# TheCacophonyProject/audio-analysis

Measured on AMD Instinct MI355X. Metric: audio-seconds classified/sec/GPU on 60 s mono; max|delta logit| vs CPU ref, higher is better.
Workload: dtype bf16x3; 1 GPU; config2: 64 windows/step (39 of clip A + 25 of clip B, 60 s 48 kHz mono), htk log-mel n_fft 4096 hop 640 160 mel + model1 CNN; model=model1, global_batch=64, seq_len=144000, parallelism=dp1, pipeline=2 batches in flight on 2 streams, clip_pairs=4 resident clip pairs in rotation, one per step

## Files before the change

audio-analysis_amd/csrc/aa_cnn.hip:

```cpp
#include "aa_common.h"

#include <cmath>
#include <cstdlib>
#include <cstring>
#include <string>
#include <type_traits>
#include <vector>

namespace aa {

typedef __attribute__((ext_vector_type(8))) __bf16 bf16x8;
typedef __attribute__((ext_vector_type(4))) float f32x4;
typedef __attribute__((ext_vector_type(2))) float f32x2;
typedef __attribute__((ext_vector_type(16))) float f32x16;
typedef __bf16 bf16;
struct fp8 {
    uint8_t v;
};
struct bf16x3 {};

template <typename T>
struct Prec {
    using L = T;
    using G = T;
// ... 819 lines not shown
            for (int o = 0; o < 8; ++o)
                if (o < nc) best[o] = fmaxf(best[o], apply_act(acc[o] + bias[c0 + o], act, alpha));
        }
    TO* dst = out + ((size_t)(n * Hout + oh) * Wout + ow) * cout + c0;
    for (int o = 0; o < nc; ++o) dst[o] = to_t<TO>(best[o]);
}

template <typename TI>
__global__ __launch_bounds__(256) void pool_dense(const TI* __restrict__ in, int HW, int C,
                                                  const float* __restrict__ w, const float* __restrict__ b, int U,
                                                  int sigmoid, float* __restrict__ logits, float* __restrict__ probs) {
    extern __shared__ float mx[];
    const int n = blockIdx.x;
    const TI* src = in + (size_t)n * HW * C;
    for (int c = threadIdx.x; c < C; c += blockDim.x) {
        float m = -INFINITY;
        for (int p = 0; p < HW; ++p) m = fmaxf(m, to_f(src[(size_t)p * C + c]));
        mx[c] = m;
    }
    __syncthreads();
    for (int u = threadIdx.x; u < U; u += blockDim.x) {
        float v;
        if (w) {
            v = 0.f;
            for (int c = 0; c < C; ++c) v = fmaf(mx[c], w[(size_t)c * U + u], v);
            v += b[u];
        } else {
            v = mx[u];
        }
        logits[(size_t)n * U + u] = v;
        if (probs) probs[(size_t)n * U + u] = sigmoid ? 1.f / (1.f + expf(-v)) : v;
    }
}

__global__ void track_mean(const float* __restrict__ probs, int n_models, long long model_stride, int L,
                           const int* __restrict__ wb, const int* __restrict__ wc,
                           float* __restrict__ out) {
    const int t = blockIdx.x;
    const int c = threadIdx.x;
    if (c >= L) return;
    constexpr int U = 40;
    float acc = 0.f;
    const int n = wc[t];
    const float* base = probs + (size_t)wb[t] * L + c;
    for (int w0 = 0; w0 < n; w0 += U) {
        float m[U];
#pragma unroll
        for (int u = 0; u < U; ++u) m[u] = 0.f;
        for (int k = 0; k < n_models; ++k) {
            float v[U];
#pragma unroll
            for (int u = 0; u < U; ++u) v[u] = base[k * model_stride + (size_t)min(w0 + u, n - 1) * L];
#pragma unroll
            for (int u = 0; u < U; ++u) m[u] = __fadd_rn(m[u], v[u]);
        }
#pragma unroll
        for (int u = 0; u < U; ++u)
            if (w0 + u < n) acc = __fadd_rn(acc, __fdiv_rn(m[u], (float)n_models));
    }
    out[(size_t)t * L + c] = n > 0 ? __fdiv_rn(acc, (float)n) : NAN;
}

}

#include "aa_conv_x3.h"
#include "aa_conv_wg.h"
#include "aa_gconv.h"
#include "aa_conv_tail.h"

namespace aa {

template <int MODE>
__global__ void stage_decode(const void* __restrict__ src, float* __restrict__ dst, size_t total, int cout) {
    for (size_t i = (size_t)blockIdx.x * blockDim.x + threadIdx.x; i < total; i += (size_t)gridDim.x * blockDim.x) {
        float v;
        if (MODE == 0) {
            v = static_cast<const float*>(src)[i];
        } else if (MODE == 1) {
            v = __uint_as_float((uint32_t) static_cast<const uint16_t*>(src)[i] << 16);
        } else if (MODE == 2) {
            const uint32_t b = static_cast<const uint8_t*>(src)[i];
            const int e = (b >> 3) & 15, m = b & 7;
            const float a = (e == 15 && m == 7) ? __uint_as_float(0x7fc00000u)
                            : e == 0            ? ldexpf((float)m, -9)
                                                : ldexpf((float)(8 + m), e - 10);
            v = (b & 0x80) ? -a : a;
        } else {
            const size_t pix = i / (size_t)cout;
            const int c = (int)(i - pix * (size_t)cout);
            const uint16_t* h = static_cast<const uint16_t*>(src) + pix * (size_t)cout * 2 + (size_t)(c >> 5) * 64 + (c & 31);
            v = __uint_as_float((uint32_t)h[0] << 16) + __uint_as_float((uint32_t)h[32] << 16);
        }
        dst[i] = v;
    }
}

}

#include "aa_cnn_plan.h"

namespace aa {

template <typename Launch>
static int launch_tuned(const Stage& s, const Stage* first, int n, const void* kernel, size_t lds, bool window32,
                        int pool, int th, int tw, int bn, Launch&& launch) {
    if (window32)
        AA_CHECK((double)s.Hin * s.Win * s.cin * 4 < 2147483647.0, AA_ERR_UNSUPPORTED,
                 "conv %s: one window's activations exceed 2 GiB", s.name.c_str());
    FirstConv fc{};
    if (first) {
        const float slope = first->act == ACT_LEAKY ? first->alpha : first->act == ACT_RELU ? 0.f : 1.f;
        fc = FirstConv{(const float*)first->d_w, first->d_b, first->act, slope, first->has_mag,
                       first->mag_exp, first->Hin, first->Win, s.lm_f16};
    }
    AA_CHECK(lds <= 160 * 1024, AA_ERR_UNSUPPORTED, "conv %s: %zu B LDS", s.name.c_str(), lds);
    AA_DYN_LDS(kernel, lds);
    const int tiles_h = (s.Hout * pool + th - 1) / th;
    const int tiles_w = (s.Wout * pool + tw - 1) / tw;
    launch(dim3(tiles_h * tiles_w, s.cout_pad / bn, n), tiles_w, fc);
    AA_LAUNCH_CHECK();
    return AA_OK;
}

template <typename T, int KH, int KW, int CIN, int WM, int WN, int MF, int NF, int POOL, int TH, int TW,
          bool FUSED = false, bool EBF16 = false, int OCC = 0>
static int launch_mfma(const Stage& s, const void* in, void* out, int n, hipStream_t st,
                       const Stage* first = nullptr) {
    auto k = conv_mfma<T, KH, KW, CIN, WM, WN, MF, NF, POOL, TH, TW, FUSED, 0, EBF16, OCC>;
    constexpr int BN = WN * NF * 16;
    const size_t lds = conv_lds_bytes<T, KH, KW, CIN, BN, TH, TW, FUSED, EBF16>();
    using GT = typename Prec<T>::G;
    using LT = typename Prec<T>::L;
    return launch_tuned(s, FUSED ? first : nullptr, n, (const void*)k, lds, false, POOL, TH, TW, BN,
                        [&](dim3 grid, int tiles_w, const FirstConv& fc) {
        hipLaunchKernelGGL(k, grid, dim3(WM * WN * 64), lds, st, (const GT*)in, s.Hin, s.Win, (const LT*)s.d_w, s.d_b,
                           (GT*)out, s.Hout, s.Wout, s.cout, tiles_w, s.act, s.alpha, fc);
    });
}

template <int KH, int KW, int CIN, int WM, int WN, int MF, int NF, int POOL, int TH, int TW, bool RING, bool AJIT,
          int OCC, bool FUSED, bool IN_SPLIT, bool OUT_SPLIT>
static int launch_x3(const Stage& s, const void* in, void* out, int n, hipStream_t st, const Stage* first) {
    auto k = conv_x3<KH, KW, CIN, WM, WN, MF, NF, POOL, TH, TW, FUSED, 0, RING, AJIT, OCC, IN_SPLIT, OUT_SPLIT>;
    constexpr int BN = WN * NF * 16;
    const size_t lds = x3_lds_bytes<KH, KW, CIN, BN, TH, TW, FUSED, RING>();
    return launch_tuned(s, FUSED ? first : nullptr, n, (const void*)k, lds, true, POOL, TH, TW, BN,
                        [&](dim3 grid, int tiles_w, const FirstConv& fc) {
        hipLaunchKernelGGL(k, grid, dim3(WM * WN * 64), lds, st, (const float*)in, s.Hin, s.Win, (const bf16*)s.d_w,
                           s.d_b, (float*)out, s.Hout, s.Wout, s.cout, tiles_w, s.act, s.alpha, fc);
    });
}

template <int KH, int CIN, int WM, int WN, int MF, int NF, int POOL, int TH, int TW, int OCC, int WO, int NPASS,
          int BD, bool IN_SPLIT, bool OUT_SPLIT>
static int launch_wg(const Stage& s, const void* in, void* out, int n, hipStream_t st) {
    auto k = conv_wg<KH, CIN, WM, WN, MF, NF, POOL, TH, TW, OCC, IN_SPLIT, OUT_SPLIT, 0, WO, NPASS, BD>;
    constexpr int BN = WN * NF * 16;
    const size_t lds = wg_lds_bytes<KH, BN, TH, TW, WO, NPASS, WN>();
    return launch_tuned(s, nullptr, n, (const void*)k, lds, true, POOL, TH, TW, BN,
                        [&](dim3 grid, int tiles_w, const FirstConv&) {
        hipLaunchKernelGGL(k, grid, dim3(WM * WN * 64), lds, st, (const float*)in, s.Hin, s.Win, (const bf16*)s.d_w,
                           s.d_b, (float*)out, s.Hout, s.Wout, s.cout, tiles_w, s.act, s.alpha);
    });
}

template <bool CAN_FUSE, typename F>
static int dispatch_split(const Stage& s, F&& f) {
    using Y = std::true_type;
    using N = std::false_type;
    if constexpr (CAN_FUSE) {
        if (s.fused_first) return s.out_split ? f(Y{}, N{}, Y{}) : f(Y{}, N{}, N{});
    }
    if (s.in_split) return s.out_split ? f(N{}, Y{}, Y{}) : f(N{}, Y{}, N{});
    return s.out_split ? f(N{}, N{}, Y{}) : f(N{}, N{}, N{});
}

template <typename T>
static int launch_stage(const Model& m, const Stage& s, const void* in, void* out, float* logits,
                        float* probs, int n, hipStream_t st, const Stage* first, float* tmp) {
    using GT = typename Prec<T>::G;
    if (s.kind == ST_SMALL) {
        dim3 grid((s.Hc * s.Wc + 255) / 256, n);
        hipLaunchKernelGGL((conv_small<GT, 3, 3, 32>), grid, dim3(256), 0, st, (const float*)in, s.Hin,
                           s.Win, (const float*)s.d_w, s.d_b, s.has_mag, s.mag_exp, (GT*)out, s.Hc, s.Wc,
                           s.act, s.alpha);
        AA_LAUNCH_CHECK();
        return AA_OK;
    }
    if (s.kind == ST_GCONV) {
        if constexpr (!is_split<T>()) {
            set_error("%s: the runtime-shaped MFMA conv is split-bf16 only", s.name.c_str());
            return AA_ERR_UNSUPPORTED;
        } else {
            const ConvGeom g{s.Hin, s.Win, s.cin, s.Hc, s.Wc, s.cout, s.kh, s.kw, 1, 1, 0, 0, s.cin_pad};
            const bool pooled = s.ph > 1 || s.pw > 1;
            float* conv_out = pooled ? tmp : static_cast<float*>(out);
            const int gact_ = s.act == ACT_LEAKY ? GACT_LEAKY : s.act == ACT_RELU ? GACT_RELU : GACT_NONE;
            hipLaunchKernelGGL((gconv_x3t<2, 2, 2, 2>), dim3((s.Hc * s.Wc + 63) / 64, s.cout_pad / 64, n), dim3(256), 0, st,
                               (const float*)in, (const uint16_t*)s.d_w, s.d_b, conv_out, g, s.cout_pad, gact_,
                               s.alpha, nullptr, nullptr);
            AA_LAUNCH_CHECK();
            if (pooled) {
                const size_t items = (size_t)s.Hout * s.Wout * s.cout;
                hipLaunchKernelGGL(gpool2d, dim3((unsigned)((items + 255) / 256), n), dim3(256), 0, st, tmp,
                                   (float*)out, s.Hc, s.Wc, s.cout, s.Hout, s.Wout, s.ph, s.pw, s.ph, s.pw, 0, 0, 0,
                                   GACT_NONE, 0.f);
                AA_LAUNCH_CHECK();
            }
            return AA_OK;
        }
    }
    if (s.kind == ST_GENERIC) {
        if constexpr (is_fp8<T>()) {
            set_error("%s: no fp8 kernel for this shape", s.name.c_str());
            return AA_ERR_UNSUPPORTED;
        } else {
            dim3 grid((s.Hout * s.Wout + 255) / 256, (s.cout + 7) / 8, n);
            if (s.is_first) {
                hipLaunchKernelGGL((conv_generic<float, GT>), grid, dim3(256), 0, st, (const float*)in, s.Hin,
                                   s.Win, s.cin, (const float*)s.d_w, s.d_b, s.kh, s.kw, s.cout, s.ph, s.pw, s.Hout,
                                   s.Wout, s.act, s.alpha, s.has_mag, s.mag_exp, (GT*)out);
            } else {
                hipLaunchKernelGGL((conv_generic<GT, GT>), grid, dim3(256), 0, st, (const GT*)in, s.Hin, s.Win,
                                   s.cin, (const float*)s.d_w, s.d_b, s.kh, s.kw, s.cout, s.ph, s.pw, s.Hout,
                                   s.Wout, s.act, s.alpha, 0, 1.f, (GT*)out);
            }
            AA_LAUNCH_CHECK();
            return AA_OK;
        }
    }
    if (s.kind == ST_POOLDENSE) {
        hipLaunchKernelGGL((pool_dense<GT>), dim3(n), dim3(256), (size_t)s.cin * sizeof(float), st, (const GT*)in,
                           s.Hin * s.Win, s.cin, (const float*)s.d_w, s.d_b, s.cout, s.sigmoid, logits, probs);
        AA_LAUNCH_CHECK();
        return AA_OK;
    }
    if (s.kind == ST_HEAD && s.tail) {
        if constexpr (is_split<T>()) {
            const Stage& c = *first;
            const int tiles_h = (c.Hc + TAIL_TH - 1) / TAIL_TH, tiles_w = (c.Wc + TAIL_TW - 1) / TAIL_TW;
            auto k = conv_tail_x3<1, 3, 128, AA_TAIL_MF, TAIL_TH, TAIL_TW>;
            constexpr size_t lds = tail_lds_bytes<1, 3, 128, TAIL_TH, TAIL_TW>();
            AA_DYN_LDS(k, lds);
            float* part = static_cast<float*>(out);
            hipLaunchKernelGGL(k, dim3(tiles_h * tiles_w, 1, n), dim3(TAIL_NW * 64), lds, st, (const float*)in, c.Hin,
                               c.Win, (const bf16*)c.d_w, c.d_b, c.Hc, c.Wc, tiles_w, c.act, c.alpha,
                               (const bf16*)s.d_tw, part);
            AA_LAUNCH_CHECK();
            hipLaunchKernelGGL(head_final, dim3(n), dim3(64), 0, st, part, tiles_h * tiles_w, 32, s.d_b, s.cout, s.act,
                               s.alpha, s.sigmoid, logits, probs, (const float*)nullptr);
            AA_LAUNCH_CHECK();
            return AA_OK;
        } else {
            set_error("%s: the fused tail is split-bf16 only", s.name.c_str());
            return AA_ERR_UNSUPPORTED;
        }
    }
    if (s.kind == ST_HEAD) {
        const int HW = s.Hin * s.Win, parts = (HW + 63) / 64;
        float* part = static_cast<float*>(out);
        const float* hsc = is_fp8<T>() ? s.d_b + s.cout_pad : nullptr;
        hipLaunchKernelGGL((conv_head<GT, 1, 2>), dim3(n, parts, s.cout_pad / 32), dim3(256), 0, st, (const GT*)in,
                           HW, s.cin, (const GT*)s.d_w, s.d_b, s.cout, s.act, s.alpha, s.sigmoid, logits, probs, part,
                           hsc);
        AA_LAUNCH_CHECK();
        hipLaunchKernelGGL(head_final, dim3(n), dim3(s.cout <= 64 ? 64 : 256), 0, st, part, parts, s.cout_pad, s.d_b,
                           s.cout, s.act, s.alpha, s.sigmoid, logits, probs, hsc);
        AA_LAUNCH_CHECK();
        return AA_OK;
    }
    if (s.fused_first) {
        AA_CHECK(s.kh == 3 && s.kw == 3 && s.cin == 32 && s.pool == 3, AA_ERR_UNSUPPORTED,
                 "no fused first-layer kernel for %s", s.name.c_str());
    }
    if constexpr (is_split<T>()) {
        if (s.wg) {
#define AA_LAUNCHW(KH, CIN, POOL, WM, WN, MF, NF, TH, TW, OCC, WO, NPASS, BD)                                    \
            if (s.kh == KH && s.cin == CIN && s.pool == POOL)                                                    \
                return dispatch_split<false>(s, [&](auto, auto is, auto os) {                                    \
                    return launch_wg<KH, CIN, WM, WN, MF, NF, POOL, TH, TW, OCC, WO, NPASS, BD, decltype(is)::value, \
                                     decltype(os)::value>(s, in, out, n, st);                                    \
                });
            AA_WG_CFGS(AA_LAUNCHW)
#undef AA_LAUNCHW
            set_error("conv %dx%d cin %d pool %d: no Winograd kernel instantiation", s.kh, s.kw, s.cin, s.pool);
            return AA_ERR_UNSUPPORTED;
        }
#define AA_LAUNCH3(KH, KW, CIN, POOL, WM, WN, MF, NF, TH, TW, RING, AJIT, OCC)                                   \
        if (s.kh == KH && s.kw == KW && s.cin == CIN && s.pool == POOL)                                          \
            return dispatch_split<CIN == 32 && KH == 3 && KW == 3>(s, [&](auto fu, auto is, auto os) {           \
                return launch_x3<KH, KW, CIN, WM, WN, MF, NF, POOL, TH, TW, RING, AJIT, OCC, decltype(fu)::value, \
                                 decltype(is)::value, decltype(os)::value>(s, in, out, n, st, first);            \
            });
        AA_X3_CFGS(AA_LAUNCH3)
#undef AA_LAUNCH3
        set_error("conv %dx%d cin %d pool %d: no split-bf16 kernel instantiation", s.kh, s.kw, s.cin, s.pool);
        return AA_ERR_UNSUPPORTED;
    }
#define AA_LAUNCH(T_, KH, KW, CIN, POOL, WM, WN, MF, NF, TH, TW, EB, OCC)                                        \
    if constexpr (std::is_same<T, T_>::value) {                                                          \
        if (s.kh == KH && s.kw == KW && s.cin == CIN && s.pool == POOL) {                                \
            if (s.fused_first) {                                                                         \
                if constexpr (CIN == 32 && KH == 3 && KW == 3)                                           \
                    return launch_mfma<T, KH, KW, CIN, WM, WN, MF, NF, POOL, TH, TW, true, EB, OCC>(s, in, out, \
                                                                                              n, st, first); \
            } else {                                                                                     \
                return launch_mfma<T, KH, KW, CIN, WM, WN, MF, NF, POOL, TH, TW, false, EB, OCC>(s, in, out, n, st); \
            }                                                                                            \
        }                                                                                                \
    }
    AA_CONV_CFGS(AA_LAUNCH)
#undef AA_LAUNCH
    set_error("conv %dx%d cin %d pool %d: no kernel instantiation", s.kh, s.kw, s.cin, s.pool);
    return AA_ERR_UNSUPPORTED;
}

static void free_model(Model* m) {
    if (!m) return;
    m->timer.release();
    if (m->uploaded)
        for (auto& s : m->st) {
            (void)hipFree(s.d_w);
            (void)hipFree(s.d_b);
            (void)hipFree(s.d_tw);
        }
    delete m;
}

static int upload_model(Model* m) {
    m->uploaded = true;
    auto put = [](void** d, const void* h, size_t bytes) {
        hipError_t e = hipMalloc(d, bytes ? bytes : 4);
        if (e == hipSuccess && bytes) e = hipMemcpy(*d, h, bytes, hipMemcpyHostToDevice);
        return e;
    };
    for (Stage& s : m->st) {
        hipError_t e = s.h_w.empty() ? hipSuccess : put(&s.d_w, s.h_w.data(), s.h_w.size());
        if (e == hipSuccess) e = put((void**)&s.d_b, s.h_b.data(), sizeof(float) * s.h_b.size());
        AA_CHECK(e == hipSuccess, AA_ERR_HIP, "aa_model_create: layer %d: %s", s.layer_end, hipGetErrorString(e));
        if (!s.h_tw.empty()) e = put(&s.d_tw, s.h_tw.data(), s.h_tw.size());
        AA_CHECK(e == hipSuccess, AA_ERR_HIP, "aa_model_create: %s", hipGetErrorString(e));
        std::vector<uint8_t>().swap(s.h_w);
        std::vector<uint8_t>().swap(s.h_tw);
        std::vector<float>().swap(s.h_b);
    }
    return AA_OK;
}

template <typename T>
static int run_stages_t(Model* m, const void* x, int n, int last_stage, float* logits, float* probs, void* workspace,
                        hipStream_t st, bool timed, const void** last_out) {
    const size_t es = prec_bytes(m->prec);
    char* buf[2] = {static_cast<char*>(workspace),
                    static_cast<char*>(workspace) + align_up(m->act_elems[0] * es * n, 256)};
    float* tmp = reinterpret_cast<float*>(buf[1] + align_up(m->act_elems[1] * es * n, 256));
    const void* in = x;
    for (int k = 0; k <= last_stage; ++k) {
        const Stage& s = m->st[k];
        if (s.skipped) continue;
        void* out = buf[(s.tail ? k - 1 : k) % 2];
        const Stage* first = (s.fused_first || s.tail) ? &m->st[k - 1] : nullptr;
        hipEvent_t e0 = nullptr;
        int rc = timed ? m->timer.begin(k, st, &e0) : AA_OK;
        if (rc != AA_OK) return rc;
        rc = launch_stage<T>(*m, s, in, out, logits, probs, n, st, first, tmp);
        if (rc != AA_OK) return rc;
        rc = m->timer.end(k, st, e0);
        if (rc != AA_OK) return rc;
        in = out;
    }
    if (last_out) *last_out = in;
    return AA_OK;
}

static int run_stages(Model* m, const void* x, int n, int last_stage, float* logits, float* probs, void* workspace,
                      hipStream_t st, bool timed, const void** last_out = nullptr) {
    switch (m->prec) {
        case AA_PREC_BF16: return run_stages_t<bf16>(m, x, n, last_stage, logits, probs, workspace, st, timed, last_out);
        case AA_PREC_FP8: return run_stages_t<fp8>(m, x, n, last_stage, logits, probs, workspace, st, timed, last_out);
        case AA_PREC_BF16X3: return run_stages_t<bf16x3>(m, x, n, last_stage, logits, probs, workspace, st, timed, last_out);
        default: return run_stages_t<float>(m, x, n, last_stage, logits, probs, workspace, st, timed, last_out);
    }
}

}

using namespace aa;

extern "C" int aa_model_plan(const aa_layer* layers, int32_t n_layers, const float* blob, int64_t blob_len,
                             int32_t in_h, int32_t in_w, int32_t in_c, int32_t precision, void** model) {
    AA_CHECK(model, AA_ERR_INVALID, "aa_model_create: null argument");
    Model* m = nullptr;
    const int rc = plan_model(layers, n_layers, blob, blob_len, in_h, in_w, in_c, precision, &m);
    if (rc == AA_OK) *model = m;
    return rc;
}

extern "C" int aa_model_create(const aa_layer* layers, int32_t n_layers, const float* blob, int64_t blob_len,
                               int32_t in_h, int32_t in_w, int32_t in_c, int32_t precision, void** model) {
    void* m = nullptr;
    int rc = aa_model_plan(layers, n_layers, blob, blob_len, in_h, in_w, in_c, precision, model ? &m : nullptr);
    if (rc != AA_OK) return rc;
    rc = upload_model(static_cast<Model*>(m));
    if (rc != AA_OK) {
        free_model(static_cast<Model*>(m));
        return rc;
    }
    *model = m;
    return AA_OK;
}

extern "C" int aa_model_stage_image(const void* model, int32_t stage, int32_t which, void* buf, size_t cap,
                                    size_t* len) {
    const Model* m = static_cast<const Model*>(model);
    AA_CHECK(m && len && stage >= 0 && stage < (int)m->st.size() && which >= 0 && which <= 2, AA_ERR_INVALID,
             "aa_model_stage_image: bad argument");
    AA_CHECK(!m->uploaded, AA_ERR_UNSUPPORTED,
             "aa_model_stage_image: the host images are released once a model is created; plan it (aa_model_plan)");
    const Stage& s = m->st[stage];
    const void* src = which == 0 ? (const void*)s.h_w.data() : which == 1 ? (const void*)s.h_b.data() : s.h_tw.data();
    *len = which == 0 ? s.h_w.size() : which == 1 ? s.h_b.size() * sizeof(float) : s.h_tw.size();
    if (!buf) return AA_OK;
    AA_CHECK(cap >= *len, AA_ERR_INVALID, "aa_model_stage_image: buffer %zu < %zu", cap, *len);
    if (*len) memcpy(buf, src, *len);
    return AA_OK;
}

extern "C" int aa_model_destroy(void* model) {
    free_model(static_cast<Model*>(model));
    return AA_OK;
}

extern "C" int aa_model_n_outputs(const void* model) {
    return model ? static_cast<const Model*>(model)->L : -1;
// ... 132 lines not shown
```

audio-analysis_amd/csrc/aa_cnn_tiles.h:

```cpp
#pragma once

namespace aa {

#define AA_CONV_CFGS(X)                                     \
    X(bf16, 3, 3, 32, 3, 4, 1, 6, 2, 18, 21, true, 0)          \
    X(bf16, 3, 3, 32, 1, 2, 2, 4, 2, 8, 16, true, 0)           \
    X(bf16, 3, 3, 64, 1, 2, 2, 4, 2, 8, 16, true, 0)           \
    X(bf16, 9, 3, 64, 3, 4, 2, 6, 4, 39, 9, true, 0)           \
    X(bf16, 1, 3, 128, 1, 2, 4, 5, 2, 7, 20, false, 0)         \
    X(fp8, 3, 3, 32, 3, 4, 1, 6, 2, 12, 30, true, 0)           \
    X(fp8, 3, 3, 32, 1, 2, 2, 4, 2, 8, 16, true, 0)            \
    X(fp8, 3, 3, 64, 1, 4, 1, 3, 4, 12, 16, true, 0)           \
    X(fp8, 9, 3, 64, 3, 4, 2, 6, 4, 21, 18, true, 0)           \
    X(fp8, 1, 3, 128, 1, 2, 4, 5, 2, 7, 20, true, 0)           \
    X(float, 3, 3, 32, 3, 2, 2, 9, 1, 6, 48, false, 0)         \
    X(float, 3, 3, 32, 1, 1, 4, 9, 1, 6, 24, false, 0)         \
    X(float, 3, 3, 64, 1, 1, 4, 9, 1, 6, 24, false, 0)         \
    X(float, 9, 3, 64, 3, 1, 4, 7, 1, 3, 33, false, 0)         \
    X(float, 1, 3, 128, 1, 2, 2, 5, 1, 6, 24, false, 0)

#ifdef AA_X3_ALT
#define AA_X3_CFGS(X) AA_X3_ALT(X)
#else
#define AA_X3_CFGS(X)                                 \
    X(3, 3, 32, 3, 4, 1, 4, 2, 12, 21, 0, 1, 0)       \
    X(3, 3, 32, 1, 4, 2, 3, 2, 10, 18, 1, 0, 4)       \
    X(3, 3, 64, 1, 2, 2, 3, 2, 12, 8, 1, 1, 0)        \
    X(9, 3, 64, 3, 2, 2, 4, 2, 21, 6, 0, 1, 4)        \
    X(1, 3, 128, 1, 2, 2, 3, 2, 7, 12, 1, 1, 0)
#endif

#ifdef AA_WG_ALT
#define AA_WG_CFGS(X) AA_WG_ALT(X)
#else
#define AA_WG_CFGS(X) X(9, 64, 3, 1, 4, 3, 1, 39, 6, 0, 6, 1, 2)
#endif

#ifndef AA_TAIL_TW
#define AA_TAIL_TW 5
#define AA_TAIL_MF 5
#endif
constexpr int TAIL_TH = 13, TAIL_TW = AA_TAIL_TW;

static int wg_bn(int kh, int kw, int cin, int pool) {
#define AA_WBN(KH, CIN, POOL, WM, WN, MF, NF, TH, TW, OCC, WO, NPASS, BD) \
    if (kw == 3 && kh == KH && cin == CIN && pool == POOL) return WN * NF * 16;
    AA_WG_CFGS(AA_WBN)
#undef AA_WBN
    return 0;
}
static void wg_form(int kh, int cin, int pool, int* wo, int* npass) {
#define AA_WFORM(KH, CIN, POOL, WM, WN, MF, NF, TH, TW, OCC, WO, NPASS, BD) \
    if (kh == KH && cin == CIN && pool == POOL) { *wo = WO; *npass = NPASS; return; }
    AA_WG_CFGS(AA_WFORM)
#undef AA_WFORM
    *wo = 0;
    *npass = 1;
}

template <typename T>
constexpr int prec_of() {
    return is_split<T>() ? AA_PREC_BF16X3 : sizeof(T) == 1 ? AA_PREC_FP8 : sizeof(T) == 2 ? AA_PREC_BF16 : AA_PREC_F32;
}

static int mfma_bn(int prec, int kh, int kw, int cin, int pool) {
    if (prec == AA_PREC_BF16X3 && wg_bn(kh, kw, cin, pool)) return wg_bn(kh, kw, cin, pool);
#define AA_BN(T_, KH, KW, CIN, POOL, WM, WN, MF, NF, TH, TW, EB, OCC)                                       \
    if (prec_of<T_>() == prec && kh == KH && kw == KW && cin == CIN && pool == POOL) \
        return WN * NF * 16;
    AA_CONV_CFGS(AA_BN)
#undef AA_BN
#define AA_BN3(KH, KW, CIN, POOL, WM, WN, MF, NF, TH, TW, RING, AJIT, OCC)                                               \
    if (prec == AA_PREC_BF16X3 && kh == KH && kw == KW && cin == CIN && pool == POOL) return WN * NF * 16;
    AA_X3_CFGS(AA_BN3)
#undef AA_BN3
    return 0;
}

}
```

audio-analysis_amd/csrc/aa_conv_wg.h:

```cpp
#pragma once

#include <type_traits>

namespace aa {

__host__ __device__ constexpr float wg_bt(int wo, int e, int t) {
    constexpr float b2[4][4] = {{1, 0, -1, 0}, {0, 1, 1, 0}, {0, -1, 1, 0}, {0, 1, 0, -1}};
    constexpr float b3[5][5] = {{2, -1, -2, 1, 0}, {0, -2, -1, 1, 0}, {0, 2, -3, 1, 0}, {0, -1, 0, 1, 0},
                                {0, 2, -1, -2, 1}};
    constexpr float b4[6][6] = {{4, 0, -5, 0, 1, 0},  {0, -4, -4, 1, 1, 0}, {0, 4, -4, -1, 1, 0},
                                {0, -2, -1, 2, 1, 0}, {0, 2, -1, -2, 1, 0}, {0, 4, 0, -5, 0, 1}};
    constexpr float b6[8][8] = {{-1, 0, 5.25f, 0, -5.25f, 0, 1, 0},         {0, 1, 1, -4.25f, -4.25f, 1, 1, 0},
                                {0, -1, 1, 4.25f, -4.25f, -1, 1, 0},        {0, 0.5f, 0.25f, -2.5f, -1.25f, 2, 1, 0},
                                {0, -0.5f, 0.25f, 2.5f, -1.25f, -2, 1, 0},  {0, 2, 4, -2.5f, -5, 0.5f, 1, 0},
                                {0, -2, 4, 2.5f, -5, -0.5f, 1, 0},          {0, -1, 0, 5.25f, 0, -5.25f, 0, 1}};
    return wo == 2 ? b2[e][t] : wo == 3 ? b3[e][t] : wo == 4 ? b4[e][t] : b6[e][t];
}
__host__ __device__ constexpr float wg_at(int wo, int k, int e) {
    constexpr float a2[2][4] = {{1, 1, 1, 0}, {0, 1, -1, -1}};
    constexpr float a3[3][5] = {{1, 1, 1, 1, 0}, {0, 1, -1, 2, 0}, {0, 1, 1, 4, 1}};
    constexpr float a4[4][6] = {{1, 1, 1, 1, 1, 0}, {0, 1, -1, 2, -2, 0}, {0, 1, 1, 4, 4, 0}, {0, 1, -1, 8, -8, 1}};
    constexpr float a6[6][8] = {{1, 1, 1, 1, 1, 1, 1, 0},
                                {0, 1, -1, 2, -2, 0.5f, -0.5f, 0},
                                {0, 1, 1, 4, 4, 0.25f, 0.25f, 0},
                                {0, 1, -1, 8, -8, 0.125f, -0.125f, 0},
                                {0, 1, 1, 16, 16, 0.0625f, 0.0625f, 0},
                                {0, 1, -1, 32, -32, 0.03125f, -0.03125f, 1}};
    return wo == 2 ? a2[k][e] : wo == 3 ? a3[k][e] : wo == 4 ? a4[k][e] : a6[k][e];
}
static inline double wg_g(int wo, int e, int k) {
    static const double g2[4][3] = {{1, 0, 0}, {0.5, 0.5, 0.5}, {0.5, -0.5, 0.5}, {0, 0, 1}};
    static const double g3[5][3] = {{0.5, 0, 0},
                                    {-0.5, -0.5, -0.5},
                                    {-1.0 / 6, 1.0 / 6, -1.0 / 6},
                                    {1.0 / 6, 1.0 / 3, 2.0 / 3},
                                    {0, 0, 1}};
    static const double g4[6][3] = {{0.25, 0, 0},
                                    {-1.0 / 6, -1.0 / 6, -1.0 / 6},
                                    {-1.0 / 6, 1.0 / 6, -1.0 / 6},
                                    {1.0 / 24, 1.0 / 12, 1.0 / 6},
                                    {1.0 / 24, -1.0 / 12, 1.0 / 6},
                                    {0, 0, 1}};
    static const double g6[8][3] = {{-1, 0, 0},
                                    {-2.0 / 9, -2.0 / 9, -2.0 / 9},
                                    {-2.0 / 9, 2.0 / 9, -2.0 / 9},
                                    {1.0 / 90, 1.0 / 45, 2.0 / 45},
                                    {1.0 / 90, -1.0 / 45, 2.0 / 45},
                                    {32.0 / 45, 16.0 / 45, 8.0 / 45},
                                    {32.0 / 45, -16.0 / 45, 8.0 / 45},
                                    {0, 0, 1}};
    return wo == 2 ? g2[e][k] : wo == 3 ? g3[e][k] : wo == 4 ? g4[e][k] : g6[e][k];
}

template <int B, int E, typename Fn>
__device__ __forceinline__ void wg_static_for(Fn&& f) {
    if constexpr (B < E) {
        f(std::integral_constant<int, B>{});
        wg_static_for<B + 1, E>(f);
    }
}

template <int KH, int TH, int TW, int WO, int NPASS>
__host__ __device__ constexpr size_t wg_patch_bytes() {
    return (size_t)((WO + 2) / NPASS) * (TH + KH - 1) * (TW / WO) * 128;
}

#ifndef AA_WG_EPH
#define AA_WG_EPH 2
#endif
__host__ __device__ constexpr int wg_eph(int BN, int WN) {
    return (AA_WG_EPH > 1 && WN % AA_WG_EPH == 0 && BN / AA_WG_EPH >= 32) ? AA_WG_EPH : 1;
}
template <int KH, int BN, int TH, int TW, int WO, int NPASS, int WN = 1>
constexpr size_t wg_lds_bytes() {
    const size_t main = wg_patch_bytes<KH, TH, TW, WO, NPASS>();
    const size_t epi = (size_t)TH * TW * (BN / wg_eph(BN, WN)) * 4;
    return main > epi ? main : epi;
}

constexpr int wg_psh(int wo) { return wo == 4 ? 2 : wo == 3 ? 0 : 1; }

template <int WO, int PPS, int E0, int NP, int PV, int NTHR, int ITEMS, typename Load4>
__device__ __forceinline__ void wg_stage(char* patch, int oh0, int ow0, int Hin, int Win, int g, Load4&& load4) {
    constexpr int A = WO + 2;
    for (int idx = threadIdx.x; idx < ITEMS; idx += NTHR) {
        const int v = idx >> 3, cq = idx & 7;
        const int R = v / NP, jp = v - (v / NP) * NP;
        const int gh = min(oh0 + R, Hin - 1);
        float4 d[A];
#pragma unroll
        for (int c = 0; c < A; ++c) d[c] = load4(gh, min(ow0 + WO * jp + c, Win - 1), g, cq);
        const int unit = (((cq >> 1) + v) & 7) << 4;
        float4 u6[WO == 6 ? 8 : 1];
        if constexpr (WO == 6) {
            auto f = [&](auto get, auto put) {
                const float d0 = get(d[0]), d1 = get(d[1]), d2 = get(d[2]), d3 = get(d[3]);
                const float d4 = get(d[4]), d5 = get(d[5]), d6 = get(d[6]), d7 = get(d[7]);
                put(0, fmaf(5.25f, d2 - d4, d6 - d0));
                put(7, fmaf(5.25f, d3 - d5, d7 - d1));
                const float a12 = fmaf(-4.25f, d4, d2 + d6), b12 = fmaf(-4.25f, d3, d1 + d5);
                put(1, a12 + b12);
                put(2, a12 - b12);
                const float a34 = fmaf(-1.25f, d4, fmaf(0.25f, d2, d6));
                const float b34 = fmaf(2.f, d5, fmaf(-2.5f, d3, 0.5f * d1));
                put(3, a34 + b34);
                put(4, a34 - b34);
                const float a56 = fmaf(-5.f, d4, fmaf(4.f, d2, d6));
                const float b56 = fmaf(0.5f, d5, fmaf(-2.5f, d3, 2.f * d1));
                put(5, a56 + b56);
                put(6, a56 - b56);
            };
            f([](const float4& x) { return x.x; }, [&](int e, float y) { u6[e].x = y; });
            f([](const float4& x) { return x.y; }, [&](int e, float y) { u6[e].y = y; });
            f([](const float4& x) { return x.z; }, [&](int e, float y) { u6[e].z = y; });
            f([](const float4& x) { return x.w; }, [&](int e, float y) { u6[e].w = y; });
        }
#pragma unroll
        for (int el = 0; el < PPS; ++el) {
            float4 u = make_float4(0.f, 0.f, 0.f, 0.f);
            if constexpr (WO == 6) u = u6[E0 + el];
#pragma unroll
            for (int t = 0; t < (WO == 6 ? 0 : A); ++t) {
                const float b = wg_bt(WO, E0 + el, t);
                if (b == 0.f) continue;
                if (b == 1.f) {
                    u.x += d[t].x; u.y += d[t].y; u.z += d[t].z; u.w += d[t].w;
                } else if (b == -1.f) {
                    u.x -= d[t].x; u.y -= d[t].y; u.z -= d[t].z; u.w -= d[t].w;
                } else {
                    u.x = fmaf(b, d[t].x, u.x); u.y = fmaf(b, d[t].y, u.y);
                    u.z = fmaf(b, d[t].z, u.z); u.w = fmaf(b, d[t].w, u.w);
                }
            }
            uint32_t h0, l0, h1, l1;
            split2(u.x, u.y, h0, l0);
            split2(u.z, u.w, h1, l1);
            const int a = (el * PV + v) * 128 + unit + (cq & 1) * 8;
            *reinterpret_cast<uint2*>(patch + a) = make_uint2(h0, h1);
            *reinterpret_cast<uint2*>(patch + (a ^ 64)) = make_uint2(l0, l1);
        }
    }
}

template <int KH, int CIN, int WM, int WN, int MF, int NF, int POOL, int TH, int TW, int OCC = 0,
          bool IN_SPLIT = false, bool OUT_SPLIT = false, int DIAG = 0, int WO = 2, int NPASS = 1, int BD = 2>
__global__ __launch_bounds__(WM * WN * 64)
__attribute__((amdgpu_waves_per_eu(OCC ? OCC : 1, OCC ? OCC : 8)))
void conv_wg(const float* __restrict__ in, int Hin, int Win, const bf16* __restrict__ wt,
             const float* __restrict__ bias, float* __restrict__ out, int Hout, int Wout, int cout_store,
             int tiles_w, int act, float alpha) {
    typedef __attribute__((ext_vector_type(4))) __bf16 bf16x4;
    constexpr int A = WO + 2;
    constexpr int PPS = A / NPASS;
    static_assert(WO >= 2 && WO <= 6 && WO != 5, "F(2|3|4|6, 3)");
    static_assert(A % NPASS == 0, "whole passes");
    static_assert(BD >= 2 && ((A / NPASS) % 2 != 0 || (A / NPASS) % BD == 0), "B ring depth divides the pass");
    static_assert(TW % WO == 0 && TH % POOL == 0 && TW % POOL == 0, "group- and pool-aligned tile");
    constexpr int NP = TW / WO;
    constexpr int TP = TH * NP;
    static_assert(TP <= WM * MF * 16, "tile covered by the waves' fragments");
    static_assert(CIN % 32 == 0, "C_in multiple of 32");
    constexpr int NTHR = WM * WN * 64;
    constexpr int BN = WN * NF * 16;
    constexpr int PH = TH + KH - 1;
    constexpr int PV = PH * NP;
    constexpr int NG = CIN / 32;
    constexpr int NSTEP = NG * NPASS * KH * PPS;
    constexpr int SLICE = BN * 64;
    extern __shared__ __attribute__((aligned(16))) char smem[];
    char* patch = smem;

    const BlockPos bp = x3_block<true>();
    const int n = bp.n, cb = bp.cb;
    const int th = bp.tile / tiles_w, tw = bp.tile - (bp.tile / tiles_w) * tiles_w;
    const int oh0 = th * TH, ow0 = tw * TW;
    const int wave = __builtin_amdgcn_readfirstlane(threadIdx.x >> 6);
    const int lane = threadIdx.x & 63;
    const int wm = wave % WM, wn = wave / WM;
    const int q = lane >> 4;

    int abase[MF], aph[MF];
#pragma unroll
    for (int i = 0; i < MF; ++i) {
        int p = (wm * MF + i) * 16 + (lane & 15);
        if (p >= TP) p = max(p - 16 * ((p - TP) / 16 + 1), 0);
        abase[i] = p * 128;
        aph[i] = p + q;
    }
    int bofs[NF];
#pragma unroll
    for (int j = 0; j < NF; ++j) {
        const int row = wn * NF * 16 + j * 16 + (lane & 15);
        bofs[j] = row * 128 + (((q + row) & 7) << 4);
    }
    const size_t step_stride = (size_t)gridDim.y * SLICE;
    const __amdgpu_buffer_rsrc_t wrs = x3_wrsrc(wt);

    f32x4 acc[A][MF][NF];
#pragma unroll
    for (int e = 0; e < A; ++e)
#pragma unroll
        for (int i = 0; i < MF; ++i)
#pragma unroll
            for (int j = 0; j < NF; ++j) acc[e][i][j] = f32x4{0.f, 0.f, 0.f, 0.f};

    struct BSet {
        bf16x8 h[NF], l[NF];
    };
    BSet Bq[BD];
    auto read_b = [&](BSet& b, int s) {
        const int soff = __builtin_amdgcn_readfirstlane((int)((cb * SLICE + s * step_stride) * 2));
#pragma unroll
        for (int j = 0; j < NF; ++j) {
            b.h[j] = x3_wload(wrs, bofs[j], soff);
            b.l[j] = x3_wload(wrs, bofs[j] ^ 64, soff);
        }
    };
    auto step = [&](auto bc, int s, int kh, auto ec, auto elc) {
        constexpr int e = decltype(ec)::value;
        constexpr int el = decltype(elc)::value;
        constexpr int b = decltype(bc)::value;
        BSet& cur = Bq[b];
        if (s + BD - 1 < NSTEP) read_b(Bq[(b + BD - 1) % BD], s + BD - 1);
        const int pofs = el * PV * 128 + kh * NP * 128, tv = kh * NP;
        bf16x8 h2[2], l2[2];
        auto rd = [&](int i, int k) {
            const int a = pofs + abase[i] + (((aph[i] + tv) & 7) << 4);
            h2[k] = *reinterpret_cast<const bf16x8*>(patch + a);
            l2[k] = *reinterpret_cast<const bf16x8*>(patch + (a ^ 64));
        };
        rd(0, 0);
        if constexpr (AA_PIN_WG & 1) __builtin_amdgcn_sched_barrier(0);
#pragma unroll
        for (int i = 0; i < MF; ++i) {
            if (i + 1 < MF) rd(i + 1, (i + 1) & 1);
            if constexpr (AA_PIN_WG & 2) __builtin_amdgcn_sched_barrier(0);
#pragma unroll
            for (int j = 0; j < NF; ++j) {
                acc[e][i][j] = __builtin_amdgcn_mfma_f32_16x16x32_bf16(cur.h[j], h2[i & 1], acc[e][i][j], 0, 0, 0);
                acc[e][i][j] = __builtin_amdgcn_mfma_f32_16x16x32_bf16(cur.l[j], h2[i & 1], acc[e][i][j], 0, 0, 0);
                acc[e][i][j] = __builtin_amdgcn_mfma_f32_16x16x32_bf16(cur.h[j], l2[i & 1], acc[e][i][j], 0, 0, 0);
            }
        }
    };

    const __amdgpu_buffer_rsrc_t ars = x3_wrsrc(reinterpret_cast<const char*>(in) + (size_t)n * Hin * Win * CIN * 4);
    constexpr int wbase = 0;
    auto load4 = [&](int gh, int gw, int g, int cq) -> float4 {
        const int pix = gh * Win + gw;
        if constexpr (IN_SPLIT) {
            const int o = pix * (CIN * 4) + g * 128 + cq * 8;
            const bf16x4 h = __builtin_bit_cast(bf16x4, __builtin_amdgcn_raw_buffer_load_b64(ars, o, wbase, 0));
            const bf16x4 l = __builtin_bit_cast(bf16x4, __builtin_amdgcn_raw_buffer_load_b64(ars, o + 64, wbase, 0));
            return make_float4((float)h[0] + (float)l[0], (float)h[1] + (float)l[1], (float)h[2] + (float)l[2],
                               (float)h[3] + (float)l[3]);
        } else {
            return __builtin_bit_cast(float4, __builtin_amdgcn_raw_buffer_load_b128(ars, (pix * CIN + g * 32 + cq * 4) * 4,
                                                                                     wbase, 0));
        }
    };

#pragma unroll
    for (int k = 0; k < BD - 1; ++k)
        if (k < NSTEP) read_b(Bq[k], k);
    wg_static_for<0, NG>([&](auto gc) {
        constexpr int g = decltype(gc)::value;
        wg_static_for<0, NPASS>([&](auto pc) {
            constexpr int pass = decltype(pc)::value;
            if (g > 0 || pass > 0) __syncthreads();
            wg_stage<WO, PPS, pass * PPS, NP, PV, NTHR, (DIAG & 1) ? 0 : PV * 8>(patch, oh0, ow0, Hin, Win, g, load4);
            __syncthreads();
            if constexpr (AA_WG_PRIO > 0) __builtin_amdgcn_s_setprio(AA_WG_PRIO);
            if constexpr ((DIAG & 2) == 0) {
                if constexpr (PPS % 2 == 0) {
                    for (int kh = 0; kh < KH; ++kh) {
                        const int s0 = ((g * NPASS + pass) * KH + kh) * PPS;
                        wg_static_for<0, PPS>([&](auto elc) {
                            constexpr int el = decltype(elc)::value;
                            constexpr std::integral_constant<int, pass * PPS + el> ec{};
                            step(std::integral_constant<int, el % BD>{}, s0 + el, kh, ec, elc);
                        });
                    }
                } else {
                    constexpr int sb = (g * NPASS + pass) * KH * PPS;
                    wg_static_for<0, KH * PPS>([&](auto sc) {
                        constexpr int si = decltype(sc)::value;
                        constexpr int kh = si / PPS, el = si % PPS;
                        constexpr std::integral_constant<int, pass * PPS + el> ec{};
                        constexpr std::integral_constant<int, el> elc{};
                        step(std::integral_constant<int, (sb + si) % BD>{}, sb + si, kh, ec, elc);
                    });
                }
            }
            if constexpr (AA_WG_PRIO > 0) __builtin_amdgcn_s_setprio(0);
        });
    });
    __syncthreads();

    constexpr int PSH = wg_psh(WO);
    constexpr int EH = wg_eph(BN, WN), WNE = WN / EH, BNE = BN / EH;
    float* E = reinterpret_cast<float*>(smem);
#pragma unroll
    for (int h = 0; h < EH; ++h) {
        if (h > 0) __syncthreads();
        if (wn / WNE == h) {
#pragma unroll
            for (int j = 0; j < NF; ++j) {
                const int u = (wn % WNE) * NF * 4 + j * 4 + q;
#pragma unroll
                for (int i = 0; i < MF; ++i) {
                    const int p = (wm * MF + i) * 16 + (lane & 15);
                    if (p < TP) {
                        const int r = p / NP, jp = p - (p / NP) * NP;
                        const int px = r * TW + WO * jp;
#pragma unroll
                        for (int k = 0; k < WO; ++k) {
                            f32x4 y = f32x4{0.f, 0.f, 0.f, 0.f};
#pragma unroll
                            for (int e = 0; e < A; ++e) {
                                const float c = wg_at(WO, k, e);
                                if (c == 0.f) continue;
                                if (c == 1.f) y += acc[e][i][j];
                                else if (c == -1.f) y -= acc[e][i][j];
                                else y += c * acc[e][i][j];
                            }
                            *reinterpret_cast<float4*>(E + x3_eoff<BNE, PSH>(px + k, u)) =
                                make_float4(y[0], y[1], y[2], y[3]);
                        }
                    }
                }
            }
        }
        __syncthreads();
        x3_store<TH, TW, POOL, BNE, NTHR, OUT_SPLIT, false, PSH>(E, bias, out, n, cb * EH + h, oh0, ow0, Hout, Wout,
                                                                cout_store, act, alpha);
    }
}

}
```

Baseline: 267,100 audio-s/s.

## Add sliding-window A-operand reuse with DPP row shifts in Winograd conv

Adds a SLIDE mode to the Winograd conv kernel. Each lane now owns MF consecutive output rows instead of strided rows, and the A fragments for successive kh taps are produced by shifting the previous rows with DPP row_shl instead of being re-read from LDS. The B-weight ring is walked in an order that matches, the ring depth goes from 2 to 4, and the epilogue pixel mapping changes to the new row ownership. The aim is to cut LDS reads per MFMA in the 9x3 layer. The cost is more registers for the extra A set and deeper B ring, which could lower occupancy, and DPP lane shifts that must be correct at the row edges.

```diff
diff --git a/audio-analysis_amd/csrc/aa_cnn.hip b/audio-analysis_amd/csrc/aa_cnn.hip
--- a/audio-analysis_amd/csrc/aa_cnn.hip
+++ b/audio-analysis_amd/csrc/aa_cnn.hip
@@ -995,9 +995,9 @@
 }
 
 template <int KH, int CIN, int WM, int WN, int MF, int NF, int POOL, int TH, int TW, int OCC, int WO, int NPASS,
-          int BD, bool IN_SPLIT, bool OUT_SPLIT>
+          int BD, int SLIDE, bool IN_SPLIT, bool OUT_SPLIT>
 static int launch_wg(const Stage& s, const void* in, void* out, int n, hipStream_t st) {
-    auto k = conv_wg<KH, CIN, WM, WN, MF, NF, POOL, TH, TW, OCC, IN_SPLIT, OUT_SPLIT, 0, WO, NPASS, BD>;
+    auto k = conv_wg<KH, CIN, WM, WN, MF, NF, POOL, TH, TW, OCC, IN_SPLIT, OUT_SPLIT, 0, WO, NPASS, BD, SLIDE>;
     constexpr int BN = WN * NF * 16;
     const size_t lds = wg_lds_bytes<KH, BN, TH, TW, WO, NPASS, WN>();
     return launch_tuned(s, nullptr, n, (const void*)k, lds, true, POOL, TH, TW, BN,
@@ -1118,11 +1118,11 @@
     }
     if constexpr (is_split<T>()) {
         if (s.wg) {
-#define AA_LAUNCHW(KH, CIN, POOL, WM, WN, MF, NF, TH, TW, OCC, WO, NPASS, BD)                                    \
+#define AA_LAUNCHW(KH, CIN, POOL, WM, WN, MF, NF, TH, TW, OCC, WO, NPASS, BD, SLIDE)                             \
             if (s.kh == KH && s.cin == CIN && s.pool == POOL)                                                    \
                 return dispatch_split<false>(s, [&](auto, auto is, auto os) {                                    \
-                    return launch_wg<KH, CIN, WM, WN, MF, NF, POOL, TH, TW, OCC, WO, NPASS, BD, decltype(is)::value, \
-                                     decltype(os)::value>(s, in, out, n, st);                                    \
+                    return launch_wg<KH, CIN, WM, WN, MF, NF, POOL, TH, TW, OCC, WO, NPASS, BD, SLIDE,           \
+                                     decltype(is)::value, decltype(os)::value>(s, in, out, n, st);               \
                 });
             AA_WG_CFGS(AA_LAUNCHW)
 #undef AA_LAUNCHW
diff --git a/audio-analysis_amd/csrc/aa_cnn_tiles.h b/audio-analysis_amd/csrc/aa_cnn_tiles.h
--- a/audio-analysis_amd/csrc/aa_cnn_tiles.h
+++ b/audio-analysis_amd/csrc/aa_cnn_tiles.h
@@ -33,7 +33,7 @@
 #ifdef AA_WG_ALT
 #define AA_WG_CFGS(X) AA_WG_ALT(X)
 #else
-#define AA_WG_CFGS(X) X(9, 64, 3, 1, 4, 3, 1, 39, 6, 0, 6, 1, 2)
+#define AA_WG_CFGS(X) X(9, 64, 3, 1, 4, 3, 1, 39, 6, 0, 6, 1, 4, 9)
 #endif
 
 #ifndef AA_TAIL_TW
@@ -43,14 +43,14 @@
 constexpr int TAIL_TH = 13, TAIL_TW = AA_TAIL_TW;
 
 static int wg_bn(int kh, int kw, int cin, int pool) {
-#define AA_WBN(KH, CIN, POOL, WM, WN, MF, NF, TH, TW, OCC, WO, NPASS, BD) \
+#define AA_WBN(KH, CIN, POOL, WM, WN, MF, NF, TH, TW, OCC, WO, NPASS, BD, SLIDE) \
     if (kw == 3 && kh == KH && cin == CIN && pool == POOL) return WN * NF * 16;
     AA_WG_CFGS(AA_WBN)
 #undef AA_WBN
     return 0;
 }
 static void wg_form(int kh, int cin, int pool, int* wo, int* npass) {
-#define AA_WFORM(KH, CIN, POOL, WM, WN, MF, NF, TH, TW, OCC, WO, NPASS, BD) \
+#define AA_WFORM(KH, CIN, POOL, WM, WN, MF, NF, TH, TW, OCC, WO, NPASS, BD, SLIDE) \
     if (kh == KH && cin == CIN && pool == POOL) { *wo = WO; *npass = NPASS; return; }
     AA_WG_CFGS(AA_WFORM)
 #undef AA_WFORM
diff --git a/audio-analysis_amd/csrc/aa_conv_wg.h b/audio-analysis_amd/csrc/aa_conv_wg.h
--- a/audio-analysis_amd/csrc/aa_conv_wg.h
+++ b/audio-analysis_amd/csrc/aa_conv_wg.h
@@ -142,8 +142,22 @@
     }
 }
 
+template <int KH, int PPS>
+__host__ __device__ constexpr int wg_slide_s(int v) {
+    const int pi = v / (KH * PPS), t = v % (KH * PPS);
+    return (pi * KH + t % KH) * PPS + t / KH;
+}
+__device__ __forceinline__ bf16x8 wg_row_shl1(bf16x8 x) {
+    typedef __attribute__((ext_vector_type(4))) int i32x4;
+    i32x4 v = __builtin_bit_cast(i32x4, x);
+#pragma unroll
+    for (int k = 0; k < 4; ++k) v[k] = __builtin_amdgcn_update_dpp(0, v[k], 0x101, 0xf, 0xf, true);
+    return __builtin_bit_cast(bf16x8, v);
+}
+
 template <int KH, int CIN, int WM, int WN, int MF, int NF, int POOL, int TH, int TW, int OCC = 0,
-          bool IN_SPLIT = false, bool OUT_SPLIT = false, int DIAG = 0, int WO = 2, int NPASS = 1, int BD = 2>
+          bool IN_SPLIT = false, bool OUT_SPLIT = false, int DIAG = 0, int WO = 2, int NPASS = 1, int BD = 2,
+          int SLIDE = 0>
 __global__ __launch_bounds__(WM * WN * 64)
 __attribute__((amdgpu_waves_per_eu(OCC ? OCC : 1, OCC ? OCC : 8)))
 void conv_wg(const float* __restrict__ in, int Hin, int Win, const bf16* __restrict__ wt,
@@ -154,7 +168,7 @@
     constexpr int PPS = A / NPASS;
     static_assert(WO >= 2 && WO <= 6 && WO != 5, "F(2|3|4|6, 3)");
     static_assert(A % NPASS == 0, "whole passes");
-    static_assert(BD >= 2 && ((A / NPASS) % 2 != 0 || (A / NPASS) % BD == 0), "B ring depth divides the pass");
+    static_assert(BD >= 2 && (SLIDE > 0 || (A / NPASS) % 2 != 0 || (A / NPASS) % BD == 0), "B ring depth divides the pass");
     static_assert(TW % WO == 0 && TH % POOL == 0 && TW % POOL == 0, "group- and pool-aligned tile");
     constexpr int NP = TW / WO;
     constexpr int TP = TH * NP;
@@ -166,6 +180,8 @@
     constexpr int PV = PH * NP;
     constexpr int NG = CIN / 32;
     constexpr int NSTEP = NG * NPASS * KH * PPS;
+    static_assert(SLIDE == 0 || (NP == 1 && WM == 1 && PH <= MF * 16),
+                  "sliding A: one column group per row, one wave over the plane's rows");
     constexpr int SLICE = BN * 64;
     extern __shared__ __attribute__((aligned(16))) char smem[];
     char* patch = smem;
@@ -244,6 +260,63 @@
         }
     };
 
+    struct ASet {
+        bf16x8 h, l;
+    };
+    ASet Ar[2][MF + 1];
+    const int srow = MF * (lane & 15);
+    auto slide_ofs = [&](int m) {
+        const int row = min(srow + m, PH - 1);
+        return row * 128 + (((row + q) & 7) << 4);
+    };
+    int sofs[MF], sofl[MF];
+#pragma unroll
+    for (int i = 0; i < MF; ++i) {
+        sofs[i] = slide_ofs(i);
+        sofl[i] = sofs[i] ^ 64;
+    }
+    auto rd_slide = [&](ASet& r, int el, int m) {
+        const int ah = m < MF ? sofs[m < MF ? m : 0] : slide_ofs(m);
+        const int al = m < MF ? sofl[m < MF ? m : 0] : ah ^ 64;
+        r.h = *reinterpret_cast<const bf16x8*>(patch + el * PV * 128 + ah);
+        r.l = *reinterpret_cast<const bf16x8*>(patch + el * PV * 128 + al);
+    };
+    auto slide_step = [&](auto bc, auto vc, auto tc, auto ec) {
+        constexpr int e = decltype(ec)::value;
+        constexpr int b = decltype(bc)::value;
+        constexpr int v = decltype(vc)::value;
+        constexpr int t = decltype(tc)::value;
+        constexpr int S = SLIDE > 0 ? SLIDE : 1, RL = (KH + S - 1) / S;
+        constexpr int el = t / KH, kh = t % KH, gen = (el * RL + kh / S) & 1;
+        constexpr bool more = t + 1 < KH * PPS;
+        constexpr int nel = (t + 1) / KH, nkh = (t + 1) % KH, ngen = (nel * RL + nkh / S) & 1;
+        constexpr bool reload = more && nkh % S == 0;
+        BSet& cur = Bq[b];
+        if constexpr (v + BD - 1 < NSTEP) read_b(Bq[(b + BD - 1) % BD], wg_slide_s<KH, PPS>(v + BD - 1));
+        if constexpr (t == 0) {
+#pragma unroll
+            for (int i = 0; i < MF; ++i) rd_slide(Ar[gen][i], el, i);
+        }
+        if constexpr (AA_PIN_WG & 1) __builtin_amdgcn_sched_barrier(0);
+        wg_static_for<0, MF>([&](auto ic) {
+            constexpr int i = decltype(ic)::value;
+            const ASet& a = Ar[gen][(kh + i) % (MF + 1)];
+            if constexpr (reload) rd_slide(Ar[ngen][(nkh + i) % (MF + 1)], nel, nkh + i);
+            if constexpr (AA_PIN_WG & 2) __builtin_amdgcn_sched_barrier(0);
+#pragma unroll
+            for (int j = 0; j < NF; ++j) {
+                acc[e][i][j] = __builtin_amdgcn_mfma_f32_16x16x32_bf16(cur.h[j], a.h, acc[e][i][j], 0, 0, 0);
+                acc[e][i][j] = __builtin_amdgcn_mfma_f32_16x16x32_bf16(cur.l[j], a.h, acc[e][i][j], 0, 0, 0);
+                acc[e][i][j] = __builtin_amdgcn_mfma_f32_16x16x32_bf16(cur.h[j], a.l, acc[e][i][j], 0, 0, 0);
+            }
+            if constexpr (i == 0 && more && !reload) {
+                ASet& n = Ar[gen][(kh + MF) % (MF + 1)];
+                n.h = wg_row_shl1(a.h);
+                n.l = wg_row_shl1(a.l);
+            }
+        });
+    };
+
     const __amdgpu_buffer_rsrc_t ars = x3_wrsrc(reinterpret_cast<const char*>(in) + (size_t)n * Hin * Win * CIN * 4);
     constexpr int wbase = 0;
     auto load4 = [&](int gh, int gw, int g, int cq) -> float4 {
@@ -262,7 +335,7 @@
 
 #pragma unroll
     for (int k = 0; k < BD - 1; ++k)
-        if (k < NSTEP) read_b(Bq[k], k);
+        if (k < NSTEP) read_b(Bq[k], SLIDE ? wg_slide_s<KH, PPS>(k) : k);
     wg_static_for<0, NG>([&](auto gc) {
         constexpr int g = decltype(gc)::value;
         wg_static_for<0, NPASS>([&](auto pc) {
@@ -271,7 +344,14 @@
             wg_stage<WO, PPS, pass * PPS, NP, PV, NTHR, (DIAG & 1) ? 0 : PV * 8>(patch, oh0, ow0, Hin, Win, g, load4);
             __syncthreads();
             if constexpr (AA_WG_PRIO > 0) __builtin_amdgcn_s_setprio(AA_WG_PRIO);
-            if constexpr ((DIAG & 2) == 0) {
+            if constexpr ((DIAG & 2) == 0 && SLIDE > 0) {
+                constexpr int vb = (g * NPASS + pass) * KH * PPS;
+                wg_static_for<0, KH * PPS>([&](auto tc) {
+                    constexpr int t = decltype(tc)::value;
+                    constexpr std::integral_constant<int, pass * PPS + t / KH> ec{};
+                    slide_step(std::integral_constant<int, (vb + t) % BD>{}, std::integral_constant<int, vb + t>{}, tc, ec);
+                });
+            } else if constexpr ((DIAG & 2) == 0) {
                 if constexpr (PPS % 2 == 0) {
                     for (int kh = 0; kh < KH; ++kh) {
                         const int s0 = ((g * NPASS + pass) * KH + kh) * PPS;
@@ -309,7 +389,7 @@
                 const int u = (wn % WNE) * NF * 4 + j * 4 + q;
 #pragma unroll
                 for (int i = 0; i < MF; ++i) {
-                    const int p = (wm * MF + i) * 16 + (lane & 15);
+                    const int p = SLIDE ? MF * (lane & 15) + i : (wm * MF + i) * 16 + (lane & 15);
                     if (p < TP) {
                         const int r = p / NP, jp = p - (p / NP) * NP;
                         const int px = r * TW + WO * jp;
```

Result: faster. 272,900 audio-s/s, median of 6 (+2.2%).
